# manycore-research/faceformer

Hardware: AMD Instinct MI355X
Metric: decoded edges/sec (greedy face-loop decode, pointer selections/s), 256-edge wireframes (higher is better)
Workload: dtype f32; 1 GPU; BASELINE config 2: configs/ours.yml model.num_lines=256: 1 synthetic 256-edge wireframe(s) per GPU, F=256 anchor sequences x 36 greedy steps, default-xavier synthetic weights; wireframes_per_gpu=1, edges=256, max_face_length=37, decode_steps=36, parallelism=wireframe-sharded x1, RCCL all-gather of predictions

## Files before the change

faceformer_amd/csrc/ff_common.h:

```cpp
#pragma once
#include <hip/hip_runtime.h>
#include <stdint.h>
#include <stdio.h>
#include <string.h>

#include "faceformer_hip.h"

#define FF_WAVE 64
#define FF_MAX_STREAMS 8

typedef float f32x4 __attribute__((ext_vector_type(4)));
typedef float f32x16 __attribute__((ext_vector_type(16)));

void ff_set_error(const char* fmt, ...);

#define FF_CHECK_ARG(cond, ...)           \
  do {                                    \
    if (!(cond)) {                        \
      ff_set_error(__VA_ARGS__);          \
      return FF_ERR_ARG;                  \
    }                                     \
  } while (0)

#define FF_CHECK_HIP(expr)                                                             \
// ... 57 lines not shown

size_t ff_attention_planes_stride();
bool ff_attention_x2h_ok(const ff_attn_desc& d);
int ff_attention_x2h_launch(const ff_attn_desc& d, const void* planes, long long plane_stride, hipStream_t st);

struct ff_pointer_sync {
  int* seen;
  int* arrive;
  int* host_slot;
  int host_which;
  float* next_stats;
  int logits_ready;
  const int* slot;
  int* fin;
  int fin_j, term_lo, term_hi;
};
int ff_pointer_argmax_sync(const float* p, int ldp, const float* memory, int S, int E, const unsigned char* mask,
                           const int* kv_len, const unsigned char* extra_mask, int ldextra, int B, int seqs_per_group,
                           int* next_tok, float* best, float* second, float* logprob, float* logits, int ldlogits,
                           float* next_rows, int ldnext, int* count_ge, int ge_bound, int* count_eq, int eq_value,
                           const ff_pointer_sync* sync, ff_stream_t stream);

int ff_beam_select_sync(float* logits, int ldlogits, int S, const unsigned char* mask, const int* kv_len, int groups, int width,
                        int groups_per_wireframe, const float* scores_in, float* scores_out, const int* fin_in, int* fin_out,
                        int* hist, int ldhist, int t, int* parent, int* next_tok, int term_lo, int term_hi, const float* memory,
                        int E, float* next_rows, int ldnext, int* count_ge, int ge_bound, float* next_stats, int* arrive,
                        int* host_slot, ff_stream_t stream);
int ff_beam_init(int* tok, float* score, int* fin, int* parent, int Bc, int Fc, int W, int f0, const int* num_input, int pad_tok,
                 int term_lo, int term_hi, hipStream_t st);
int ff_beam_finalize(const int* tok, const int* parent, const float* score, int Btot, int T, const int* steps_dev,
                     const int* num_input, int dedup, int F, int W, int w0, int nw, int Fc, int f0, int b0, int64_t* beams,
                     float* scores, int64_t* predict, int* seq_of_row, hipStream_t st);

int ff_forced_tokens(const int64_t* paths, int* tok, int rows, int T, int S, hipStream_t st);
int ff_forced_finalize(const int* tok, const float* lp_all, const int* greedy_all, const int* rank_all, const int* lengths, int rows,
                       int T, float* logprob, int64_t* greedy, int* rank, float* seq_logprob, hipStream_t st);
// ... 45 lines not shown
```

faceformer_amd/csrc/ff_device.h:

```cpp
#pragma once
#include "ff_common.h"

typedef float f32x2 __attribute__((ext_vector_type(2)));

#define FF_GLOBAL __attribute__((address_space(1)))
typedef unsigned long long ff_u64;

__device__ __forceinline__ f32x4 ff_ld16(const float* p) { return *reinterpret_cast<const f32x4*>(p); }
__device__ __forceinline__ f32x2 ff_ld8(const float* p) { return *reinterpret_cast<const f32x2*>(p); }
__device__ __forceinline__ float ff_ld4(const float* p) { return *p; }
__device__ __forceinline__ void ff_st16(float* p, f32x4 v) { *reinterpret_cast<f32x4*>(p) = v; }
__device__ __forceinline__ void ff_st8(float* p, f32x2 v) { *reinterpret_cast<f32x2*>(p) = v; }
__device__ __forceinline__ void ff_st4(float* p, float v) { *p = v; }
__device__ __forceinline__ int ff_ld4i(const int* p) { return *p; }
__device__ __forceinline__ void ff_st4i(int* p, int v) { *p = v; }
__device__ __forceinline__ void ff_store_tile(float* cp, int ldc, int row0, int col, int M, bool colok, const float (&v)[16]) {
  float* p = cp + (size_t)row0 * ldc + col;
  if (row0 - (row0 & 4) + 32 <= M) {
    if (colok) {
#pragma unroll
      for (int e = 0; e < 16; ++e) ff_st4(p + (size_t)((e & 3) + 8 * (e >> 2)) * ldc, v[e]);
    }
  } else {
#pragma unroll
// ... 597 lines not shown
  const float* memory; int S, E;
  const unsigned char* mask; const int* kv_len;
  const unsigned char* extra; int ldextra;
  int B, spg;
  int* next_tok; float* best; float* second; float* logits; int ldlogits;
  float* next_rows; int ldnext;
  int* count_ge; int ge_bound; int* count_eq; int eq_value;
  int* seen;
  int* arrive;
  int* host_slot;
  int host_which;
  float* next_stats;
  const int* slot;
  int* fin; int fin_j, term_lo, term_hi;
  float* logprob;
};
__device__ __forceinline__ int ff_pointer_seq(const PointerArgs& a, int b) { return a.slot ? a.slot[b] : b; }

__device__ __forceinline__ void ff_pointer_count_block(const PointerArgs& a, int b0, const int* toks, int nvalid) {
  int nge = 0, neq = 0;
  for (int i = 0; i < nvalid; ++i) {
    const int idx = toks[i];
    if (a.fin) {
      int* fp = a.fin + ff_pointer_seq(a, b0 + i);
      const int f = __hip_atomic_load(fp, __ATOMIC_RELAXED, __HIP_MEMORY_SCOPE_SYSTEM);
      if (f < a.fin_j) continue;
      if (idx >= a.term_lo && idx < a.term_hi) __hip_atomic_store(fp, a.fin_j, __ATOMIC_RELAXED, __HIP_MEMORY_SCOPE_SYSTEM);
    }
    if (a.count_ge && idx >= a.ge_bound) ++nge;
    if (a.count_eq && idx == a.eq_value) {
// ... 54 lines not shown
    const float ob1 = __shfl_xor(b1, off, FF_WAVE), ob2 = __shfl_xor(b2, off, FF_WAVE);
    const int oi1 = __shfl_xor(i1, off, FF_WAVE);
    if (LP) {
      const float om = __shfl_xor(lmax, off, FF_WAVE), os = __shfl_xor(lsum, off, FF_WAVE);
      lsum = ff_lse_merge(lmax, lsum, om, os, &lmax);
    }
    const bool other = (ob1 > b1) || (ob1 == b1 && oi1 < i1);
    const float nb2 = other ? fmaxf(ob2, b1) : fmaxf(b2, ob1);
    if (other) { b1 = ob1; i1 = oi1; }
    b2 = nb2;
  }
  if (i1 == 0x7fffffff) { i1 = 0; b1 = FILL; }
  *b1_out = b1; *b2_out = b2; *i1_out = i1; *lsum_out = lsum;
}

__device__ __forceinline__ void ff_pointer_append_row(const PointerArgs& a, int w, int b, int i1, int lane) {
  const float* src = a.memory + ((size_t)w * a.S + i1) * a.E;
  float* dst = a.next_rows + (size_t)b * a.ldnext;
  if (!a.next_stats) {
    for (int vi = lane; vi < (a.E >> 2); vi += 64)
      ff_st16(dst + vi * 4, ff_ldw16(src + vi * 4));
  } else {
    float* sdst = a.next_stats + (size_t)b * (a.E >> 5) * 2;
    for (int v0 = 0; v0 < (a.E >> 2); v0 += 64) {
      const int vi = v0 + lane;
      const bool in = vi < (a.E >> 2);
      f32x4 x = {0.f, 0.f, 0.f, 0.f};
      if (in) { x = ff_ldw16(src + vi * 4); ff_st16(dst + vi * 4, x); }
      float sm = (x.x + x.y) + (x.z + x.w);
      sm += __shfl_xor(sm, 1, FF_WAVE); sm += __shfl_xor(sm, 2, FF_WAVE); sm += __shfl_xor(sm, 4, FF_WAVE);
      const float mean = sm * (1.0f / 32.0f);
      const float d0 = x.x - mean, d1 = x.y - mean, d2 = x.z - mean, d3 = x.w - mean;
      float m2 = (d0 * d0 + d1 * d1) + (d2 * d2 + d3 * d3);
      m2 += __shfl_xor(m2, 1, FF_WAVE); m2 += __shfl_xor(m2, 2, FF_WAVE); m2 += __shfl_xor(m2, 4, FF_WAVE);
      if (in && (lane & 7) == 0) ff_st8(sdst + (vi >> 3) * 2, f32x2{mean, m2});
    }
  }
}

template <bool LP>
__device__ __forceinline__ int ff_pointer_reduce_row(const PointerArgs& a, int b, int lane) {
  float b1, b2, lsum;
  int i1;
  ff_pointer_mask_reduce<LP>(a, b, lane, &b1, &b2, &i1, &lsum);
  const int seq = ff_pointer_seq(a, b);
  if (lane == 0) {
    ff_st4i(a.next_tok + seq, i1);
    if (a.best) ff_st4(a.best + seq, b1);
    if (a.second) ff_st4(a.second + seq, b2);
    if (LP) ff_st4(a.logprob + seq, -logf(lsum));
  }
  if (a.next_rows) ff_pointer_append_row(a, b / a.spg, b, i1, lane);
  return i1;
}
```

faceformer_amd/csrc/ff_engine.hip:

```cpp
#include <chrono>
#include <cstdlib>
#include <mutex>
#include <vector>

#include "ff_common.h"
#include "ff_launch.h"

namespace {

struct Bump {
  char* base;
  size_t size, off;
  bool ok;
  Bump(void* p, size_t n) : base((char*)p), size(n), off(0), ok(true) {}
  template <typename T>
  T* take(size_t count) {
    size_t bytes = ff_align_up(count * sizeof(T), 256);
    if (off + bytes > size) { ok = false; off += bytes; return nullptr; }
    T* r = reinterpret_cast<T*>(base + off);
    off += bytes;
    return r;
  }
};

// ... 124 lines not shown
  g.row_table = d.table; g.ld_row_table = d.ldt; g.row_div = row_div; g.row_cols = d.tcols;
  g.ln_stats_out = d.st_out;
  if (split) return sk.ln(&g, d.planes, d.plane_rows, d.row0, d.st_in ? d.colsum : nullptr, st);
  return ff_gemm_f32_ln(&g, st);
}

struct Scratch {
  float *x, *y, *yq, *qkv, *o, *h, *p, *logits;
  float* lnstat;
};

struct DecodeBuffers {
  float *mem_pos, *kvc[FF_MAX_LAYERS];
  unsigned char* kvp[FF_MAX_LAYERS];
  float *x0_all, *qkv0_all;
  float* x0stat_all;
  float *projT, *pg_all, *pc_all;
  int* tok_all;
  float* lp_all;
  Scratch scr[FF_MAX_STREAMS];
  int* zeroed; size_t zeroed_count;
  int *cnt_ge, *cnt_eq;
  int *arrive;
  int *seen;
  int *cnt_tot;
  int *steps_dev;
  int *fin, *slot_all, *perm_all;
  float* bm_score;
  int *bm_fin, *bm_parent;
  float* fc_lp;
  int *fc_greedy, *fc_rank;
  float* sm_lp;
  int *sm_fin, *sm_row;
};

struct Chunk {
  int w0, nw, Fc, f0, b0, Bc, sid;
  int Fl, Bl;
  int *slot, *perm;
  float* x0;
  float* qkv0;
  float* x0stat;
  float *pg, *pc;
};

inline bool retiring(const ff_decode_params* p) { return p->variant == FF_PARALLEL && (p->flags & FF_RETIRE_FINISHED); }

inline int compact_width(const ff_decode_params* p, const int* num_input_host, int w) {
  if (p->variant != FF_PARALLEL || !(p->flags & FF_DEDUP_PAD_ANCHORS) || !num_input_host) return p->F;
  int n = num_input_host[w];
  n = n < 0 ? 0 : n;
  return n < p->F ? n + 1 : p->F;
}

void plan_chunks(const ff_decode_params* p, const int* num_input_host, int ns, std::vector<Chunk>* out, int* btot,
                 int* max_bc, int* nchunks = nullptr) {
  const int N = p->N;
// ... 64 lines not shown
  k.pinned = pc > 0 && pc < FF_PINNED_SLOTS ? pc : FF_PINNED_SLOTS;
  return k;
}

bool can_fuse_layernorm(const ff_model* m, const ff_decode_params* prm) {
  if (!(prm->flags & FF_FUSE_LAYERNORM)) return false;
  if (m->E % 64 != 0 || m->E < 128 || m->E > 512 || m->FF % 64 != 0 || m->FF < 128) return false;
  if (!m->proj_fold_w || !m->proj_fold_b) return false;
  for (int l = 0; l < m->num_dec_layers; ++l) {
    const ff_layer_weights& w = m->dec[l];
    if (!w.ln1_w || !w.ln1_b || !w.ln1_pos || !w.ln2_w || !w.ln2_b || !w.ln2_pos || !w.ln3_w || !w.ln3_b) return false;
  }
  return true;
}

size_t layout_decode(const ff_model* m, const ff_decode_params* p, const EngineKnobs& kn, size_t Btot, size_t Bch, size_t nch,
                     Bump& bp, DecodeBuffers* out, bool want_lp = false, bool beam = false, bool forced = false, bool sample = false) {
  const int E = m->E, FFd = m->FF, S = p->L + m->num_token, T = p->T;
  const int ns = plan_streams(p);
  const size_t Rmax = (size_t)(T - 1 > 0 ? T - 1 : 1) * Bch;
  DecodeBuffers b;
  memset(&b, 0, sizeof(b));
  b.mem_pos = bp.take<float>((size_t)p->N * S * E);
  for (int l = 0; l < m->num_dec_layers; ++l) b.kvc[l] = bp.take<float>((size_t)p->N * S * 2 * E);
  const bool planes = kn.x2h_attn && (m->split_kind == 1 || m->split_kind == 2) && p->x3_min_rows > 0 && S <= 288 && m->dec[0].in_proj_planes != nullptr;
  for (int l = 0; l < m->num_dec_layers; ++l)
    b.kvp[l] = planes ? bp.take<unsigned char>(ff_attention_planes_bytes(p->N, m->H)) : nullptr;
  b.x0_all = bp.take<float>((size_t)T * Btot * E);
  b.tok_all = bp.take<int>((size_t)T * Btot);
  b.qkv0_all = (p->flags & FF_REUSE_LAYER0_QKV) ? bp.take<float>((size_t)T * Btot * 3 * E) : nullptr;
  b.x0stat_all = (kn.l0_fold && (p->flags & FF_REUSE_LAYER0_QKV) && can_fuse_layernorm(m, p)) ? bp.take<float>(Btot * (size_t)(E / 32) * 2)
                                                                                 : nullptr;
  const bool pf = kn.pointer_fold && can_fuse_layernorm(m, p);
  b.projT = pf ? bp.take<float>((size_t)E * E) : nullptr;
  b.pg_all = pf ? bp.take<float>(nch * (size_t)S * E) : nullptr;
  b.pc_all = pf ? bp.take<float>(nch * (size_t)((S + 3) & ~3)) : nullptr;
  for (int s = 0; s < ns; ++s) {
    Scratch& c = b.scr[s];
    c.x = bp.take<float>(Rmax * E);
    c.y = bp.take<float>(Rmax * E);
    c.yq = bp.take<float>(Rmax * E);
    c.qkv = bp.take<float>(Rmax * 3 * E);
    c.o = bp.take<float>(Rmax * E);
    c.h = bp.take<float>(Rmax * FFd);
    c.p = bp.take<float>(Bch * E);
    c.logits = bp.take<float>(Bch * (size_t)S);
    c.lnstat = bp.take<float>(Rmax * (size_t)(E / 32 + 1) * 2);
  }
  const size_t ncnt = ff_align_up((size_t)T * nch * sizeof(int), 256) / sizeof(int);
  b.zeroed_count = 3 * ncnt + Btot;
  b.zeroed = bp.take<int>(b.zeroed_count);
// ... 47 lines not shown
  const bool prune_last = (prm->flags & FF_LAST_LAYER_LAST_ROW) != 0 && !full_rows;
  const bool fuse = step_fuses(m, prm, R);
  const int nseg = E / 32;
  const float* qpos = m->qpos_table;
  const float* qpos_new = qpos + (size_t)(t - 1) * E;
  auto proj = [&](const Proj& d) -> int { return project(m, prm, Bc, st, d); };
  const bool last_qkv_one = R <= kn.one_launch_rows;
  for (int l = 0; l < nd; ++l) {
    const ff_layer_weights& w = m->dec[l];
    const ff_mha_weights& sa = w.self_attn;
    const bool last = prune_last && (l == nd - 1);
    const float* xin = (l == 0) ? ck.x0 : buf.x;
    const float* QKV = buf.qkv;
    if (l == 0 && reuse0) {
      if (full_rows) {
      } else if (fuse && t > 1 && ck.x0stat) {
        FF_RETURN_IF(proj(Proj().in(xin + newoff * E, E).weight(w.ln1_w, E, w.ln1_b).norm(ck.x0stat)
                              .pos(w.ln1_pos + (size_t)(t - 1) * 2 * E, 2 * E, 2 * E).out(ck.qkv0 + newoff * 3 * E, 3 * E, Bc, 3 * E, E)));
      } else {
        FF_RETURN_IF(ff_layernorm(xin + newoff * E, E, w.norm1_w, w.norm1_b, m->ln_eps, buf.y, E, buf.yq, E,
                                  qpos_new, E, Bc, 1, Bc, E, st));
        FF_RETURN_IF(proj(Proj().in(buf.yq, E, buf.y, 2 * E).weight(sa.in_proj_w, E, sa.in_proj_b)
                              .out(ck.qkv0 + newoff * 3 * E, 3 * E, Bc, 3 * E, E)));
      }
      QKV = ck.qkv0;
    } else if (fuse && l > 0) {
      const bool kv_only = last && t > 1 && !last_qkv_one;
      const int c0 = kv_only ? E : 0;
      FF_RETURN_IF(proj(Proj().in(buf.x, E).weight(w.ln1_w + (size_t)c0 * E, E, w.ln1_b + c0).split(w.ln1_planes, 3 * E, c0, w.ln1_csum)
                            .norm(buf.lnstat).pos(w.ln1_pos + c0, 2 * E, 2 * E - c0).out(buf.qkv + c0, 3 * E, R, 3 * E - c0, E)));
// ... 209 lines not shown
    if (io.extra_mask || forced) prm.flags &= ~FF_DEDUP_PAD_ANCHORS;
    p = &prm;
    retire = retiring(p);
    dedup = p->variant == FF_PARALLEL && (p->flags & FF_DEDUP_PAD_ANCHORS) && io.num_input_host;
    each_eos = (p->flags & FF_STOP_EACH_EOS) != 0;
    kn = engine_knobs(p);
    return FF_OK;
  }
  int bind_chunks(void* workspace, size_t workspace_bytes) {
    const int ns_req = plan_streams(p);
    int max_bc = 0;
    if (W || R) plan_beam_chunks(p, io.num_input_host, ns_req, W ? W : R, &chunks, &Btot, &max_bc);
    else plan_chunks(p, io.num_input_host, ns_req, &chunks, &Btot, &max_bc);
    nch = (int)chunks.size();
    Bump bp(workspace, workspace_bytes);
    layout_decode(m, p, kn, (size_t)Btot, (size_t)max_bc, (size_t)nch, bp, &buf, io.logprob != nullptr, W > 0, forced != nullptr,
                  R > 0);
    if (!bp.ok) { ff_set_error("ff_decode: workspace too small (%zu needed, %zu given)", bp.off, workspace_bytes); return FF_ERR_WORKSPACE; }
    for (Chunk& c : chunks) {
      c.x0 = buf.x0_all + (size_t)T * c.b0 * E;
      c.qkv0 = buf.qkv0_all ? buf.qkv0_all + (size_t)T * c.b0 * 3 * E : nullptr;
      c.x0stat = buf.x0stat_all ? buf.x0stat_all + (size_t)c.b0 * (E / 32) * 2 : nullptr;
      const size_t ci = (size_t)(&c - chunks.data());
      const bool one = c.nw == 1 && buf.pg_all != nullptr;
      c.pg = one ? buf.pg_all + ci * (size_t)S * E : nullptr;
      c.pc = one ? buf.pc_all + ci * (size_t)((S + 3) & ~3) : nullptr;
      if (retire) { c.slot = buf.slot_all + c.b0; c.perm = buf.perm_all + c.b0; }
    }
    ns = ns_req < nch ? ns_req : nch;
    forked = ns > 1;
    lagged = (size_t)T * (size_t)nch <= (size_t)kn.pinned;
    fin_dev = buf.fin;
    slots_per_step.reserve((size_t)T);
    tot.reserve((size_t)T);
// ... 90 lines not shown
      }
    }
    FF_RETURN_IF(fork());
    bool any_pg = false;
    for (const Chunk& c : chunks) any_pg = any_pg || c.pg != nullptr;
    if (any_pg) {
      FF_RETURN_IF(ff_transpose(m->proj_fold_w, E, E, E, buf.projT, E, main_st));
      FF_RETURN_IF(fork());
      for (const Chunk& c : chunks) {
        if (!c.pg) continue;
        const float* mem_w = memory + (size_t)c.w0 * S * E;
        FF_RETURN_IF(gemm(mem_w, E, nullptr, 0, buf.projT, E, nullptr, nullptr, 0, c.pg, E, S, E, E, 0, sts[c.sid]));
        FF_RETURN_IF(gemm(mem_w, E, nullptr, 0, m->proj_fold_b, E, nullptr, nullptr, 0, c.pc, 1, S, 1, E, 0, sts[c.sid]));
      }
    }
    for (const Chunk& c : chunks) {
      if (forced) {
        FF_RETURN_IF(ff_gather_rows(memory + (size_t)c.w0 * S * E, S, E, buf.tok_all + c.b0, c.Bc, c.Fc, c.x0, E, sts[c.sid]));
        continue;
      }
      if (W) {
        FF_RETURN_IF(ff_beam_init(buf.tok_all + c.b0, buf.bm_score + c.b0, buf.bm_fin + c.b0, buf.bm_parent + c.b0, c.Bc, c.Fc / W, W,
                                  c.f0, io.num_input + c.w0, m->num_token - 1, p->term_lo, p->term_hi, sts[c.sid]));
        FF_RETURN_IF(ff_gather_rows(memory + (size_t)c.w0 * S * E, S, E, buf.tok_all + c.b0, c.Bc, c.Fc, c.x0, E, sts[c.sid]));
        continue;
      }
      if (R) {
        FF_RETURN_IF(ff_sample_init(buf.tok_all + c.b0, buf.sm_lp + c.b0, buf.sm_fin + c.b0, buf.sm_row + c.b0, c.Bc, c.Fc / R, R, c.f0,
                                    c.w0, F, io.num_input + c.w0, m->num_token - 1, p->term_lo, p->term_hi, sts[c.sid]));
        FF_RETURN_IF(ff_gather_rows(memory + (size_t)c.w0 * S * E, S, E, buf.tok_all + c.b0, c.Bc, c.Fc, c.x0, E, sts[c.sid]));
        continue;
      }
      hipLaunchKernelGGL(init_tokens_kernel, dim3(ff_cdiv(c.Bc, 256)), dim3(256), 0, sts[c.sid], buf.tok_all + c.b0,
                         c.Bc, c.Fc, c.f0, io.num_input ? io.num_input + c.w0 : nullptr, p->variant, m->num_token - 1,
                         p->tok_sos, c.slot, c.perm, c.slot ? c.Bl : 0);
      FF_CHECK_LAUNCH();
      if (c.Bl > 0)
        FF_RETURN_IF(ff_gather_rows(memory + (size_t)c.w0 * S * E, S, E, c.slot ? c.perm : buf.tok_all + c.b0, c.Bl, c.Fl, c.x0, E,
                                    sts[c.sid]));
    }
    return FF_OK;
  }
  int enqueue_step(int step) {
    const int t = step + 1;
    int nslots = 0;
    for (const Chunk& c : chunks) {
      if (c.Bl == 0) continue;
      nslots += c.Bl;
      hipStream_t st = sts[c.sid];
      const Scratch& sc = buf.scr[c.sid];
      const size_t trow = (size_t)step * ((size_t)N * F * (W ? W : (R ? R : 1))) + c.b0;
      const size_t slot = (size_t)step * nch + (size_t)(&c - chunks.data());
      const bool folded_head = c.pg != nullptr && step_fuses(m, p, (long)t * c.Bl);
      float* logits_dst = (io.trace_logits && !retire) ? io.trace_logits + trow * S : sc.logits;
      if (W) {
        FF_RETURN_IF(beam_step(c, sc, step, slot, folded_head, logits_dst, trow, st));
        continue;
      }
      if (R) {
        FF_RETURN_IF(sample_step(c, sc, step, slot, folded_head, logits_dst, st));
        continue;
      }
      ff_pointer_sync psync{each_eos ? buf.seen + c.b0 : nullptr, lagged ? buf.arrive + slot : nullptr,
                            lagged ? pool->hpin_dev + slot : nullptr, p->variant == FF_PARALLEL ? 0 : 1, c.x0stat,
                            folded_head ? 1 : 0, c.slot, retire ? fin_dev + c.b0 : nullptr, t, p->term_lo, p->term_hi};
      FF_RETURN_IF(decoder_pass(m, p, kn, buf, sc, c, c.Fl, c.Bl, io.mask, io.kv_len, t, false, nullptr, st,
                                folded_head ? logits_dst : nullptr));
      FF_RETURN_IF(ff_pointer_argmax_sync(
          folded_head ? nullptr : sc.p, E, io.memory + (size_t)c.w0 * S * E, S, E, io.mask + (size_t)c.w0 * S, io.kv_len + c.w0,
          io.extra_mask ? io.extra_mask + (size_t)c.b0 * S : nullptr, S, c.Bl, c.Fl,
          buf.tok_all + (size_t)t * Btot + c.b0, io.trace_best ? io.trace_best + trow : nullptr,
          io.trace_second ? io.trace_second + trow : nullptr,
          buf.lp_all ? buf.lp_all + (size_t)step * Btot + c.b0 : nullptr,
          logits_dst, S,
          c.x0 + (size_t)t * c.Bl * E, E, buf.cnt_ge + slot, m->num_token, buf.cnt_eq + slot, p->tok_eos,
          (each_eos || lagged || c.x0stat || folded_head || retire) ? &psync : nullptr, st));
      if (retire && io.trace_logits)
        FF_RETURN_IF(ff_permute_rows(sc.logits, c.Bl, nullptr, io.trace_logits + trow * S, c.Bc, c.slot, 1, c.Bl, S, st));
    }
    slots_per_step.push_back(nslots);
// ... 101 lines not shown
      for (int i = 0; i < nb; ++i) nhs[(size_t)i] = hs[(size_t)perm[(size_t)i]];
      if (nb > 0) {
        int* sp = pool->stage + soff;
        int* ss = sp + nb;
        soff += 2 * (size_t)nb;
        memcpy(sp, perm.data(), sizeof(int) * (size_t)nb);
        memcpy(ss, nhs.data(), sizeof(int) * (size_t)nb);
        FF_CHECK_HIP(hipMemcpyAsync(c.perm, sp, sizeof(int) * (size_t)nb, hipMemcpyHostToDevice, st));
        const Scratch& sc = buf.scr[c.sid];
        auto regather = [&](float* rows, float* scratch, int npos, int width) -> int {
          FF_RETURN_IF(ff_permute_rows(rows, c.Bl, c.perm, scratch, nb, nullptr, npos, nb, width, st));
          FF_CHECK_HIP(hipMemcpyAsync(rows, scratch, sizeof(float) * (size_t)npos * nb * width, hipMemcpyDeviceToDevice, st));
          return FF_OK;
        };
        FF_RETURN_IF(regather(c.x0, sc.x, enq + 1, E));
        if (c.qkv0) FF_RETURN_IF(regather(c.qkv0, sc.qkv, enq, 3 * E));
        if (c.x0stat) FF_RETURN_IF(regather(c.x0stat, sc.y, 1, E / 16));
        FF_CHECK_HIP(hipMemcpyAsync(c.slot, ss, sizeof(int) * (size_t)nb, hipMemcpyHostToDevice, st));
      }
      hs.swap(nhs);
      c.Fl = fl; c.Bl = nb;
    }
    return FF_OK;
  }
  int retire_at(int bound, bool drained) {
    if (fin_host) {
      const volatile int* v = fin_host;
      for (int i = 0; i < Btot; ++i) hfin[(size_t)i] = v[i];
    } else {
      FF_RETURN_IF(read_back(hfin.data(), buf.fin, (size_t)Btot, drained));
      bound = enq - 1;
// ... 157 lines not shown
    d.scale = 0.125f;
    FF_RETURN_IF(ff_attention(&d, st));
    FF_RETURN_IF(gemm(o, E, nullptr, 0, w.self_attn.out_w, E, w.self_attn.out_b, x, E, x, E, R, E, E, 0, st));
    FF_RETURN_IF(ff_layernorm(x, E, w.norm2_w, w.norm2_b, m->ln_eps, y, E, nullptr, 0, nullptr, 0, 1, 1, R, E, st));
    FF_RETURN_IF(gemm(y, E, nullptr, 0, w.lin1_w, E, w.lin1_b, nullptr, 0, hb, FFd, R, FFd, E, 1, st));
    FF_RETURN_IF(gemm(hb, FFd, nullptr, 0, w.lin2_w, FFd, w.lin2_b, x, E, x, E, R, E, FFd, 0, st));
  }
  FF_RETURN_IF(ff_layernorm(x, E, m->enc_norm_w, m->enc_norm_b, m->ln_eps, memory, E, nullptr, 0, nullptr, 0, 1, 1,
                            R, E, st));
  return FF_OK;
}

extern "C" size_t ff_decode_workspace_bytes(const ff_model* m, const ff_decode_params* p, const int* num_input_host) {
  if (!m || !p || p->N <= 0 || p->F <= 0 || p->T <= 0) return 0;
  int btot = 0, max_bc = 0, nch = 0;
  plan_chunks(p, num_input_host, 1, nullptr, &btot, &max_bc, &nch);
  Bump bp(nullptr, 0);
  return layout_decode(m, p, engine_knobs(p), (size_t)btot, (size_t)max_bc, (size_t)nch, bp, nullptr) + 256;
}

extern "C" size_t ff_decode_lp_workspace_bytes(const ff_model* m, const ff_decode_params* p, const int* num_input_host) {
  if (!m || !p || p->N <= 0 || p->F <= 0 || p->T <= 0) return 0;
  int btot = 0, max_bc = 0, nch = 0;
  plan_chunks(p, num_input_host, 1, nullptr, &btot, &max_bc, &nch);
  Bump bp(nullptr, 0);
  return layout_decode(m, p, engine_knobs(p), (size_t)btot, (size_t)max_bc, (size_t)nch, bp, nullptr, true) + 256;
}

extern "C" size_t ff_decode_beam_workspace_bytes(const ff_model* m, const ff_decode_params* p, const int* num_input_host, int width) {
  if (!m || !p || p->N <= 0 || p->F <= 0 || p->T <= 0 || width < 1 || width > 8) return 0;
  int btot = 0, max_bc = 0, nch = 0;
  plan_beam_chunks(p, num_input_host, 1, width, nullptr, &btot, &max_bc, &nch);
  Bump bp(nullptr, 0);
  return layout_decode(m, p, engine_knobs(p), (size_t)btot, (size_t)max_bc, (size_t)nch, bp, nullptr, false, true) + 256;
}

extern "C" int ff_decode(const ff_model* m, const ff_decode_params* p, const float* memory,
                         const unsigned char* mask, const int* kv_len, const int* num_input,
                         const int* num_input_host, const unsigned char* extra_mask, int64_t* predict,
                         int* steps_done, int* step_counts, float* pointer_out, float* trace_logits,
                         float* trace_best, float* trace_second, int* seq_of_row, void* workspace,
// ... 131 lines not shown
```

faceformer_amd/csrc/ff_gemm.hip:

```cpp
#include <stdlib.h>

#include "ff_common.h"
#include "ff_device.h"
#include "ff_launch.h"

namespace {


constexpr int LN_NQ = 2;
struct LnRaw { f32x2 seg[LN_NQ]; };
__device__ __forceinline__ void ff_ln_issue(const float* __restrict__ st, int nseg, int c, LnRaw& r) {
#pragma unroll
  for (int q = 0; q < LN_NQ; ++q) {
    const int sidx = c + 8 * q;
    r.seg[q] = ff_ld8(st + 2 * (sidx < nseg ? sidx : 0));
  }
}
__device__ __forceinline__ void ff_ln_finish(const LnRaw& r, int nseg, int c, float eps, float& mean, float& rstd) {
  float sm = 0.f, m2 = 0.f;
#pragma unroll
  for (int q = 0; q < LN_NQ; ++q)
    if (c + 8 * q < nseg) { sm += r.seg[q].x; m2 += r.seg[q].y; }
  sm = ff_sum8(sm);
  m2 = ff_sum8(m2);
// ... 1219 lines not shown
extern "C" int ff_set_gemm_tuning(int min_units, int two_per_cu_units, int fix_tenths, int small_max_rows) {
  FF_CHECK_ARG(min_units >= 1 && two_per_cu_units >= 1 && fix_tenths >= 0 && small_max_rows >= 0,
               "ff_set_gemm_tuning: bad arguments");
  g_sk_min_units.set(min_units);
  g_sk_two_per_cu.set(two_per_cu_units);
  g_sk_fix_tenths.set(fix_tenths);
  g_small_max_rows.set(small_max_rows);
  ff_tuning_changed();
  return FF_OK;
}

namespace {
inline long dma_min_rows() { return ff_knob(FF_K_DMA_MIN_ROWS); }
inline long dma_min_rows_n512() { return ff_knob(FF_K_DMA_MIN_ROWS_N512); }
inline long dma_min_rows_wide() { return ff_knob(FF_K_DMA_MIN_ROWS_WIDE); }
int gemm_dispatch(GemmArgs g, int batch, int tile, hipStream_t st) {
  const bool split128 = !g.A2 || (g.n_split % 128) == 0;
  if (tile == 0) tile = 7;
  if (tile == 5 && !split128) tile = 4;
  const int M = g.M, N = g.N, K = g.K;
  FFProfScope prof(FF_CAT_GEMM, 2.0 * M * N * K * batch, st);
  ff_prof_add_bytes(FF_CAT_GEMM, 4.0 * batch * ((double)M * K + (double)N * K + (double)M * N * (g.res ? 2 : 1)));
  const bool dma_ok = ff_gemm_dma_f32_ok(g, batch);
  if (tile == 11) {
    FF_CHECK_ARG(dma_ok, "ff_gemm_f32: tile 11 needs K %% 32 == 0, K >= 64, N %% 4 == 0, leading dimensions %% 4, 16-byte aligned operands, batch 1");
    return ff_gemm_dma_f32(g, st);
  }
  if (tile == 12) {
    FF_CHECK_ARG(dma_ok && (!g.A2 || (g.n_split % 64) == 0), "ff_gemm_f32: tile 12 needs what tile 11 needs");
    return ff_gemm_dma_f32(g, st, 64);
  }
  const long dmr = dma_min_rows(), dmr512 = dma_min_rows_n512(), dmrw = dma_min_rows_wide();
  const long dma_from = N <= 512 ? (dmr512 > dmr ? dmr512 : dmr) : (N >= 1536 && dmrw < dmr ? dmrw : dmr);
  if (tile == 7 && dma_ok && (long)M >= dma_from) return ff_gemm_dma_f32(g, st);
  switch (tile) {
    case 1: return launch_generic<64, 64, 32, 32>(g, batch, st);
    case 2: return launch_pipe<64, 64, 32, 32>(g, batch, st);
    case 3: return launch_persist(g, batch, st);
    case 4: return launch_pipe<128, 64, 64, 32>(g, batch, st);
    case 6: return launch_streamk(g, batch, st, 2);
    case 7:
      if (const int smr = g_small_max_rows.get(); (long)M * batch <= (N <= 512 ? smr : (smr * 3) / 4) && K >= 512 && small_ok(g))
        return launch_small(g, batch, st);
      if (batch == 1 && M >= 4096 && (K & 15) == 0 && gemm_mode(g) == 0 && (!g.A2 || (g.n_split & 63) == 0)) {
        const long t9 = (long)ff_cdiv(M, 128) * ff_cdiv(N, 64);
        const long rounds = (t9 + 511) / 512;
        if (10 * t9 >= 9 * rounds * 512) return launch_pipe<128, 64, 64, 32, 16>(g, batch, st);
      }
      return launch_streamk(g, batch, st, 0);
    case 8: FF_CHECK_ARG(small_ok(g), "ff_gemm_f32: tile 8 needs K in {128,256,512,1024}"); return launch_small(g, batch, st);
    case 9: return launch_pipe<128, 64, 64, 32, 16>(g, batch, st);
    case 10: return launch_pipe<128, 128, 64, 64, 16>(g, batch, st);
    default: return launch_pipe<128, 128, 64, 64>(g, batch, st);
  }
}
}

extern "C" int ff_gemm_f32_batched(const float* A, int lda, const float* A2, int n_split,
                                   const float* W, int ldw, const float* bias, const float* residual,
                                   int ldr, float* C, int ldc, int M, int N, int K, int act, int tile,
                                   int batch, long long stride_a, long long stride_w,
                                   long long stride_c, ff_stream_t stream) {
  if (M == 0 || N == 0 || batch == 0) return FF_OK;
  FF_CHECK_ARG(M > 0 && N > 0 && K > 0 && (K & 3) == 0, "ff_gemm_f32: bad M=%d N=%d K=%d (K %% 4)", M, N, K);
  FF_CHECK_ARG(A && W && C, "ff_gemm_f32: null operand");
  FF_CHECK_ARG((lda & 3) == 0 && (ldw & 3) == 0 && lda >= K && ldw >= K && ldc >= N,
               "ff_gemm_f32: bad leading dimensions lda=%d ldw=%d ldc=%d", lda, ldw, ldc);
  FF_CHECK_ARG(ff_aligned16(A) && ff_aligned16(W) && (!A2 || ff_aligned16(A2)),
               "ff_gemm_f32: A/A2/W must be 16-byte aligned");
  FF_CHECK_ARG(!residual || ldr >= N, "ff_gemm_f32: bad ldr");
// ... 48 lines not shown
```

faceformer_amd/csrc/ff_pointer.hip:

```cpp
#include <float.h>

#include "ff_common.h"
#include "ff_device.h"

namespace {


template <int NV, bool LP>
__device__ __forceinline__ int pointer_row(const PointerArgs& a, int b, int lane) {
  const int w = b / a.spg;
  const int nvec = a.E >> 2;
  f32x4 pv[NV];
#pragma unroll
  for (int c = 0; c < NV; ++c) {
    const int vi = lane + 64 * c;
    pv[c] = vi < nvec ? *reinterpret_cast<const f32x4*>(a.p + (size_t)b * a.ldp + vi * 4)
                      : f32x4{0.f, 0.f, 0.f, 0.f};
  }
  int kv = a.S;
  if (a.kv_len) { const int k = a.kv_len[w]; kv = k < kv ? k : kv; }
  const float* mem = a.memory + (size_t)w * a.S * a.E;
  const unsigned char* mrow = a.mask ? a.mask + (size_t)w * a.S : nullptr;
  const int seq = ff_pointer_seq(a, b);
  const unsigned char* erow = a.extra ? a.extra + (size_t)seq * a.ldextra : nullptr;
// ... 100 lines not shown
}

template <bool LP>
__global__ __launch_bounds__(256) void pointer_reduce_kernel(PointerArgs a) {
  __shared__ int s_tok[4];
  const int lane = threadIdx.x & 63;
  const int b = blockIdx.x * (blockDim.x >> 6) + (threadIdx.x >> 6);
  if (b < a.B) s_tok[threadIdx.x >> 6] = ff_pointer_reduce_row<LP>(a, b, lane);
  __syncthreads();
  if (threadIdx.x == 0) {
    const int b0 = blockIdx.x * (blockDim.x >> 6);
    ff_pointer_count_block(a, b0, s_tok, a.B - b0 < 4 ? a.B - b0 : 4);
  }
}

}

extern "C" int ff_pointer_argmax(const float* p, int ldp, const float* memory, int S, int E,
                                 const unsigned char* mask, const int* kv_len,
                                 const unsigned char* extra_mask, int ldextra, int B,
                                 int seqs_per_group, int* next_tok, float* best, float* second,
                                 float* logits, int ldlogits, float* next_rows, int ldnext,
                                 int* count_ge, int ge_bound, int* count_eq, int eq_value,
                                 ff_stream_t stream) {
  return ff_pointer_argmax_sync(p, ldp, memory, S, E, mask, kv_len, extra_mask, ldextra, B, seqs_per_group, next_tok, best,
                                second, nullptr, logits, ldlogits, next_rows, ldnext, count_ge, ge_bound, count_eq, eq_value,
                                nullptr, stream);
}

extern "C" int ff_pointer_argmax_lp(const float* p, int ldp, const float* memory, int S, int E,
// ... 9 lines not shown
}

int ff_pointer_argmax_sync(const float* p, int ldp, const float* memory, int S, int E, const unsigned char* mask,
                           const int* kv_len, const unsigned char* extra_mask, int ldextra, int B, int seqs_per_group,
                           int* next_tok, float* best, float* second, float* logprob, float* logits, int ldlogits,
                           float* next_rows, int ldnext, int* count_ge, int ge_bound, int* count_eq, int eq_value,
                           const ff_pointer_sync* sync, ff_stream_t stream) {
  if (B == 0) return FF_OK;
  FF_CHECK_ARG(B > 0 && S > 0 && E > 0 && (E & 3) == 0 && E <= 2048 && seqs_per_group > 0,
               "ff_pointer_argmax: bad sizes B=%d S=%d E=%d", B, S, E);
  const bool logits_ready = sync && sync->logits_ready;
  FF_CHECK_ARG((p || logits_ready) && memory && next_tok, "ff_pointer_argmax: null pointer");
  FF_CHECK_ARG(!logits_ready || (logits && (B % seqs_per_group) == 0), "ff_pointer_argmax: logits_ready without a logits buffer");
  FF_CHECK_ARG(!(sync && sync->next_stats) || (logits && (B % seqs_per_group) == 0 && (E & 31) == 0),
               "ff_pointer_argmax: next_stats needs the GEMM path (a logits buffer) and E %% 32 == 0");
  FF_CHECK_ARG((logits_ready && !p) || ((ldp & 3) == 0 && ff_aligned16(p)), "ff_pointer_argmax: p misaligned");
  FF_CHECK_ARG(ff_aligned16(memory), "ff_pointer_argmax: memory misaligned");
  FF_CHECK_ARG(!next_rows || ((ldnext & 3) == 0 && ff_aligned16(next_rows)), "ff_pointer_argmax: next_rows misaligned");
  FF_CHECK_ARG(!logits || ldlogits >= S, "ff_pointer_argmax: ldlogits < S");
  FF_CHECK_ARG(!extra_mask || ldextra >= S, "ff_pointer_argmax: ldextra < S");
  PointerArgs a{p, ldp, memory, S, E, mask, kv_len, extra_mask, ldextra, B, seqs_per_group,
                next_tok, best, second, logits, ldlogits, next_rows, ldnext,
                count_ge, ge_bound, count_eq, eq_value,
                sync ? sync->seen : nullptr, sync ? sync->arrive : nullptr, sync ? sync->host_slot : nullptr,
                sync ? sync->host_which : 0, sync ? sync->next_stats : nullptr,
                sync ? sync->slot : nullptr, sync ? sync->fin : nullptr, sync ? sync->fin_j : 0,
                sync ? sync->term_lo : 0, sync ? sync->term_hi : 0, logprob};
  FF_CHECK_ARG(!a.arrive || (a.host_slot && (a.host_which ? count_eq : count_ge)), "ff_pointer_argmax: counter hand-over without a counter");
  hipStream_t st = (hipStream_t)stream;
  dim3 grid(ff_cdiv(B, 4)), block(256);
  if (logits != nullptr && (B % seqs_per_group) == 0) {
    if (!logits_ready)
      FF_RETURN_IF(ff_gemm_f32_batched(p, ldp, nullptr, 0, memory, E, nullptr, nullptr, 0, logits, ldlogits,
                                       seqs_per_group, S, E, 0, 0, B / seqs_per_group,
                                       (long long)seqs_per_group * ldp, (long long)S * E,
                                       (long long)seqs_per_group * ldlogits, stream));
    FFProfScope prof(FF_CAT_POINTER, (double)B * S * 8.0, st);
    if (logprob) hipLaunchKernelGGL(pointer_reduce_kernel<true>, grid, block, 0, st, a);
    else hipLaunchKernelGGL(pointer_reduce_kernel<false>, grid, block, 0, st, a);
    FF_CHECK_LAUNCH();
    return FF_OK;
  }
// ... 15 lines not shown
```

faceformer_amd/hip/engine.py:

```python
import ctypes as C

import torch

from . import lib as _L
from .ops import SPLIT_KINDS, _dev, _p, _stream, split_weight

import operator

_VERSION_OF = operator.attrgetter("_version")

RETIRE_MIN_SHRINK = 0.125

DEFAULT_FLAGS = (_L.FF_REUSE_LAYER0_QKV | _L.FF_LAST_LAYER_LAST_ROW | _L.FF_DEDUP_PAD_ANCHORS
                 | _L.FF_FUSE_LAYERNORM)


def _kv_len_from_mask(mask_u8):
    S = mask_u8.size(1)
    idx = torch.arange(1, S + 1, device=mask_u8.device, dtype=torch.int32)
    return ((mask_u8 == 0).to(torch.int32) * idx).amax(dim=1).to(torch.int32).contiguous()


FP16_LIM = 6.0e4
ATTN_Q_SCALE = 0.125 * 1.4426950408889634


def fp16_operand_bounds(tensors, n_dec, E, weights=0.0):
    root = float(E) ** 0.5

# ... 495 lines not shown
```

faceformer_amd/hip/lib.py:

```python
import ctypes as C
import os

HERE = os.path.dirname(os.path.abspath(__file__))
LIB_PATH = os.environ.get("FF_HIP_LIB") or os.path.join(HERE, "libfaceformer_hip.so")

FF_MAX_LAYERS = 16
FF_HEAD_DIM = 64
FF_PARALLEL, FF_SEQ2SEQ = 0, 1
FF_REUSE_LAYER0_QKV, FF_LAST_LAYER_LAST_ROW, FF_RETURN_POINTER, FF_NO_STOP, FF_DEDUP_PAD_ANCHORS = 1, 2, 4, 8, 16
FF_FUSE_LAYERNORM = 32
FF_STOP_EACH_EOS = 512
FF_NO_L0_FOLD = 1024
FF_NO_POINTER_FOLD = 2048
FF_RETIRE_FINISHED = 4096
FF_ABI_VERSION = 105

fptr = C.c_void_p


class HipExtensionError(RuntimeError):
    pass


class AttnDesc(C.Structure):
    _fields_ = [
        ("q", fptr), ("k", fptr), ("v", fptr), ("o", fptr),
        ("ldq", C.c_int), ("ldk", C.c_int), ("ldv", C.c_int), ("ldo", C.c_int),
        ("num_groups", C.c_int), ("num_heads", C.c_int),
        ("nq", C.c_int),
# ... 249 lines not shown
```

include/faceformer_hip.h:

```cpp
#ifndef FACEFORMER_HIP_H
#define FACEFORMER_HIP_H

#include <stddef.h>
#include <stdint.h>

#ifdef __cplusplus
extern "C" {
#endif

typedef void* ff_stream_t;

enum ff_status {
  FF_OK = 0,
  FF_ERR_ARG = -1,
  FF_ERR_LAUNCH = -2,
  FF_ERR_WORKSPACE = -3,
  FF_ERR_NO_DEVICE = -4
};

#define FF_HEAD_DIM 64
#define FF_MAX_LAYERS 16

#define FF_ABI_VERSION 105
int ff_version(void);
// ... 194 lines not shown
int ff_encode(const ff_model* m, const float* input, const unsigned char* mask, const int* kv_len,
              int N, int L, float* memory, void* workspace, size_t workspace_bytes,
              ff_stream_t stream);

enum ff_variant { FF_PARALLEL = 0, FF_SEQ2SEQ = 1 };
enum ff_decode_flags {
  FF_REUSE_LAYER0_QKV = 1,
  FF_LAST_LAYER_LAST_ROW = 2,
  FF_RETURN_POINTER = 4,
  FF_NO_STOP = 8,
  FF_FUSE_LAYERNORM = 32,
  FF_DEDUP_PAD_ANCHORS = 16,
  FF_NO_L0_FOLD = 1024,
  FF_NO_POINTER_FOLD = 2048,
  FF_RETIRE_FINISHED = 4096,
  FF_STOP_EACH_EOS = 512
};

typedef int (*ff_stop_fn)(void* user, const int* step_counts, int num_steps);

typedef struct ff_decode_params {
  int variant;
  int N;
  int L;
  int F;
  int T;
  int chunk_wireframes;
  int chunk_seqs;
  int num_streams;
  int sync_every;
// ... 95 lines not shown
```

Baseline: 158,000 edges/s.

## Precompute layer-0 QKV table over memory rows and gather it in pointer kernel

Precomputes the layer-0 layernormed QKV projection for every memory row (S rows per wireframe) once before the greedy decode loop. The pointer argmax kernel then copies the selected row's QKV into the next step's qkv0 buffer and adds the positional term. This replaces the per-step layer-0 projection GEMM for new tokens. The cost is an upfront table GEMM, a stats kernel and extra workspace. The table is only enabled when S rows per wireframe is no more than the rows projected over all steps, and it is on by default through DEFAULT_FLAGS.

New measurement: 158,700 edges/s, median of 6. Within noise of the previous version (+0.5%).

```diff
diff --git a/faceformer_amd/csrc/ff_common.h b/faceformer_amd/csrc/ff_common.h
--- a/faceformer_amd/csrc/ff_common.h
+++ b/faceformer_amd/csrc/ff_common.h
@@ -95,12 +95,19 @@
   const int* slot;
   int* fin;
   int fin_j, term_lo, term_hi;
+  const float* tab0;
+  const float* pos0;
+  float* next_qkv;
 };
 int ff_pointer_argmax_sync(const float* p, int ldp, const float* memory, int S, int E, const unsigned char* mask,
                            const int* kv_len, const unsigned char* extra_mask, int ldextra, int B, int seqs_per_group,
                            int* next_tok, float* best, float* second, float* logprob, float* logits, int ldlogits,
                            float* next_rows, int ldnext, int* count_ge, int ge_bound, int* count_eq, int eq_value,
                            const ff_pointer_sync* sync, ff_stream_t stream);
+
+int ff_row_segment_stats(const float* x, int ldx, int rows, int E, float* stats, hipStream_t st);
+
+int ff_gemm_f32_rows_of_same_form(int M, int N, int K);
 
 int ff_beam_select_sync(float* logits, int ldlogits, int S, const unsigned char* mask, const int* kv_len, int groups, int width,
                         int groups_per_wireframe, const float* scores_in, float* scores_out, const int* fin_in, int* fin_out,
diff --git a/faceformer_amd/csrc/ff_device.h b/faceformer_amd/csrc/ff_device.h
--- a/faceformer_amd/csrc/ff_device.h
+++ b/faceformer_amd/csrc/ff_device.h
@@ -635,6 +635,7 @@
   const int* slot;
   int* fin; int fin_j, term_lo, term_hi;
   float* logprob;
+  const float* tab0; const float* pos0; float* next_qkv;
 };
 __device__ __forceinline__ int ff_pointer_seq(const PointerArgs& a, int b) { return a.slot ? a.slot[b] : b; }
 
@@ -719,6 +720,16 @@
   *b1_out = b1; *b2_out = b2; *i1_out = i1; *lsum_out = lsum;
 }
 
+__device__ __forceinline__ f32x2 ff_segment_stats(f32x4 x) {
+  float sm = (x.x + x.y) + (x.z + x.w);
+  sm += __shfl_xor(sm, 1, FF_WAVE); sm += __shfl_xor(sm, 2, FF_WAVE); sm += __shfl_xor(sm, 4, FF_WAVE);
+  const float mean = sm * (1.0f / 32.0f);
+  const float d0 = x.x - mean, d1 = x.y - mean, d2 = x.z - mean, d3 = x.w - mean;
+  float m2 = (d0 * d0 + d1 * d1) + (d2 * d2 + d3 * d3);
+  m2 += __shfl_xor(m2, 1, FF_WAVE); m2 += __shfl_xor(m2, 2, FF_WAVE); m2 += __shfl_xor(m2, 4, FF_WAVE);
+  return f32x2{mean, m2};
+}
+
 __device__ __forceinline__ void ff_pointer_append_row(const PointerArgs& a, int w, int b, int i1, int lane) {
   const float* src = a.memory + ((size_t)w * a.S + i1) * a.E;
   float* dst = a.next_rows + (size_t)b * a.ldnext;
@@ -732,13 +743,29 @@
       const bool in = vi < (a.E >> 2);
       f32x4 x = {0.f, 0.f, 0.f, 0.f};
       if (in) { x = ff_ldw16(src + vi * 4); ff_st16(dst + vi * 4, x); }
-      float sm = (x.x + x.y) + (x.z + x.w);
-      sm += __shfl_xor(sm, 1, FF_WAVE); sm += __shfl_xor(sm, 2, FF_WAVE); sm += __shfl_xor(sm, 4, FF_WAVE);
-      const float mean = sm * (1.0f / 32.0f);
-      const float d0 = x.x - mean, d1 = x.y - mean, d2 = x.z - mean, d3 = x.w - mean;
-      float m2 = (d0 * d0 + d1 * d1) + (d2 * d2 + d3 * d3);
-      m2 += __shfl_xor(m2, 1, FF_WAVE); m2 += __shfl_xor(m2, 2, FF_WAVE); m2 += __shfl_xor(m2, 4, FF_WAVE);
-      if (in && (lane & 7) == 0) ff_st8(sdst + (vi >> 3) * 2, f32x2{mean, m2});
+      const f32x2 st = ff_segment_stats(x);
+      if (in && (lane & 7) == 0) ff_st8(sdst + (vi >> 3) * 2, st);
+    }
+  }
+}
+
+__device__ __forceinline__ void ff_pointer_append_qkv0(const PointerArgs& a, int w, int b, int i1, int lane) {
+  constexpr int NB = 6;
+  const int nvec = 3 * (a.E >> 2), npos = a.E >> 1;
+  const float* src = a.tab0 + ((size_t)w * a.S + i1) * 3 * a.E;
+  float* dst = a.next_qkv + (size_t)b * 3 * a.E;
+  for (int v0 = lane; v0 < nvec; v0 += 64 * NB) {
+    f32x4 v[NB], pv[NB];
+#pragma unroll
+    for (int i = 0; i < NB; ++i) {
+      const int vi = v0 + 64 * i;
+      if (vi < nvec) v[i] = ff_ld16(src + vi * 4);
+      if (vi < npos) pv[i] = ff_ldw16(a.pos0 + vi * 4);
+    }
+#pragma unroll
+    for (int i = 0; i < NB; ++i) {
+      const int vi = v0 + 64 * i;
+      if (vi < nvec) ff_st16(dst + vi * 4, vi < npos ? v[i] + pv[i] : v[i]);
     }
   }
 }
@@ -756,5 +783,6 @@
     if (LP) ff_st4(a.logprob + seq, -logf(lsum));
   }
   if (a.next_rows) ff_pointer_append_row(a, b / a.spg, b, i1, lane);
+  if (a.tab0) ff_pointer_append_qkv0(a, b / a.spg, b, i1, lane);
   return i1;
 }
diff --git a/faceformer_amd/csrc/ff_engine.hip b/faceformer_amd/csrc/ff_engine.hip
--- a/faceformer_amd/csrc/ff_engine.hip
+++ b/faceformer_amd/csrc/ff_engine.hip
@@ -162,6 +162,7 @@
   float *mem_pos, *kvc[FF_MAX_LAYERS];
   unsigned char* kvp[FF_MAX_LAYERS];
   float *x0_all, *qkv0_all;
+  float* tab0_all;
   float* x0stat_all;
   float *projT, *pg_all, *pc_all;
   int* tok_all;
@@ -189,6 +190,7 @@
   float* x0;
   float* qkv0;
   float* x0stat;
+  float* tab0;
   float *pg, *pc;
 };
 
@@ -283,8 +285,18 @@
   return true;
 }
 
+inline bool l0_table_here(const ff_decode_params* p, const Chunk& c, int S) {
+  return (p->flags & FF_L0_TABLE) && (long)c.nw * S <= (long)c.Bc * (p->T - 1);
+}
+size_t l0_table_rows(const ff_decode_params* p, const std::vector<Chunk>& chunks, int S) {
+  size_t rows = 0;
+  for (const Chunk& c : chunks) rows += l0_table_here(p, c, S) ? (size_t)c.nw * S : 0;
+  return rows;
+}
+
 size_t layout_decode(const ff_model* m, const ff_decode_params* p, const EngineKnobs& kn, size_t Btot, size_t Bch, size_t nch,
-                     Bump& bp, DecodeBuffers* out, bool want_lp = false, bool beam = false, bool forced = false, bool sample = false) {
+                     Bump& bp, DecodeBuffers* out, bool want_lp = false, bool beam = false, bool forced = false, bool sample = false,
+                     size_t tab_rows = 0) {
   const int E = m->E, FFd = m->FF, S = p->L + m->num_token, T = p->T;
   const int ns = plan_streams(p);
   const size_t Rmax = (size_t)(T - 1 > 0 ? T - 1 : 1) * Bch;
@@ -298,12 +310,13 @@
   b.x0_all = bp.take<float>((size_t)T * Btot * E);
   b.tok_all = bp.take<int>((size_t)T * Btot);
   b.qkv0_all = (p->flags & FF_REUSE_LAYER0_QKV) ? bp.take<float>((size_t)T * Btot * 3 * E) : nullptr;
-  b.x0stat_all = (kn.l0_fold && (p->flags & FF_REUSE_LAYER0_QKV) && can_fuse_layernorm(m, p)) ? bp.take<float>(Btot * (size_t)(E / 32) * 2)
-                                                                                 : nullptr;
+  const bool l0_fold = kn.l0_fold && (p->flags & FF_REUSE_LAYER0_QKV) && can_fuse_layernorm(m, p);
+  b.x0stat_all = l0_fold ? bp.take<float>(Btot * (size_t)(E / 32) * 2) : nullptr;
   const bool pf = kn.pointer_fold && can_fuse_layernorm(m, p);
   b.projT = pf ? bp.take<float>((size_t)E * E) : nullptr;
   b.pg_all = pf ? bp.take<float>(nch * (size_t)S * E) : nullptr;
   b.pc_all = pf ? bp.take<float>(nch * (size_t)((S + 3) & ~3)) : nullptr;
+  b.tab0_all = (tab_rows && l0_fold) ? bp.take<float>(tab_rows * 3 * E) : nullptr;
   for (int s = 0; s < ns; ++s) {
     Scratch& c = b.scr[s];
     c.x = bp.take<float>(Rmax * E);
@@ -381,6 +394,7 @@
     const float* QKV = buf.qkv;
     if (l == 0 && reuse0) {
       if (full_rows) {
+      } else if (fuse && t > 1 && ck.x0stat && ck.tab0) {
       } else if (fuse && t > 1 && ck.x0stat) {
         FF_RETURN_IF(proj(Proj().in(xin + newoff * E, E).weight(w.ln1_w, E, w.ln1_b).norm(ck.x0stat)
                               .pos(w.ln1_pos + (size_t)(t - 1) * 2 * E, 2 * E, 2 * E).out(ck.qkv0 + newoff * 3 * E, 3 * E, Bc, 3 * E, E)));
@@ -620,10 +634,13 @@
     else plan_chunks(p, io.num_input_host, ns_req, &chunks, &Btot, &max_bc);
     nch = (int)chunks.size();
     Bump bp(workspace, workspace_bytes);
+    const bool greedy = !W && !R && !forced;
     layout_decode(m, p, kn, (size_t)Btot, (size_t)max_bc, (size_t)nch, bp, &buf, io.logprob != nullptr, W > 0, forced != nullptr,
-                  R > 0);
+                  R > 0, greedy ? l0_table_rows(p, chunks, S) : 0);
     if (!bp.ok) { ff_set_error("ff_decode: workspace too small (%zu needed, %zu given)", bp.off, workspace_bytes); return FF_ERR_WORKSPACE; }
+    size_t tab_off = 0;
     for (Chunk& c : chunks) {
+      if (buf.tab0_all && l0_table_here(p, c, S)) { c.tab0 = buf.tab0_all + tab_off * 3 * E; tab_off += (size_t)c.nw * S; }
       c.x0 = buf.x0_all + (size_t)T * c.b0 * E;
       c.qkv0 = buf.qkv0_all ? buf.qkv0_all + (size_t)T * c.b0 * 3 * E : nullptr;
       c.x0stat = buf.x0stat_all ? buf.x0stat_all + (size_t)c.b0 * (E / 32) * 2 : nullptr;
@@ -744,6 +761,7 @@
         FF_RETURN_IF(gemm(mem_w, E, nullptr, 0, m->proj_fold_b, E, nullptr, nullptr, 0, c.pc, 1, S, 1, E, 0, sts[c.sid]));
       }
     }
+    FF_RETURN_IF(build_l0_tables());
     for (const Chunk& c : chunks) {
       if (forced) {
         FF_RETURN_IF(ff_gather_rows(memory + (size_t)c.w0 * S * E, S, E, buf.tok_all + c.b0, c.Bc, c.Fc, c.x0, E, sts[c.sid]));
@@ -768,6 +786,27 @@
       if (c.Bl > 0)
         FF_RETURN_IF(ff_gather_rows(memory + (size_t)c.w0 * S * E, S, E, c.slot ? c.perm : buf.tok_all + c.b0, c.Bl, c.Fl, c.x0, E,
                                     sts[c.sid]));
+    }
+    return FF_OK;
+  }
+  int build_l0_tables() {
+    const int nseg = E / 32;
+    const ff_layer_weights& w = m->dec[0];
+    for (Chunk& c : chunks) {
+      if (!c.tab0) continue;
+      const int rows = c.nw * S;
+      if (c.Bl == 0 || c.Bl > rows || (long)rows > (long)c.Bl * (T - 1)) { c.tab0 = nullptr; continue; }
+      hipStream_t st = sts[c.sid];
+      const float* mem_w = io.memory + (size_t)c.w0 * S * E;
+      float* stat = buf.scr[c.sid].lnstat;
+      FF_RETURN_IF(ff_row_segment_stats(mem_w, E, rows, E, stat, st));
+      const int like = ff_gemm_f32_rows_of_same_form(c.Bl, 3 * E, E);
+      const int M = like < rows ? like : rows;
+      for (int r0 = 0; r0 < rows; r0 += M) {
+        const size_t r = (size_t)(r0 + M <= rows ? r0 : rows - M);
+        FF_RETURN_IF(project(m, p, M, st, Proj().in(mem_w + r * E, E).weight(w.ln1_w, E, w.ln1_b).norm(stat + r * nseg * 2)
+                                              .out(c.tab0 + r * 3 * E, 3 * E, M, 3 * E, E)));
+      }
     }
     return FF_OK;
   }
@@ -793,7 +832,9 @@
       }
       ff_pointer_sync psync{each_eos ? buf.seen + c.b0 : nullptr, lagged ? buf.arrive + slot : nullptr,
                             lagged ? pool->hpin_dev + slot : nullptr, p->variant == FF_PARALLEL ? 0 : 1, c.x0stat,
-                            folded_head ? 1 : 0, c.slot, retire ? fin_dev + c.b0 : nullptr, t, p->term_lo, p->term_hi};
+                            folded_head ? 1 : 0, c.slot, retire ? fin_dev + c.b0 : nullptr, t, p->term_lo, p->term_hi,
+                            c.tab0, c.tab0 ? m->dec[0].ln1_pos + (size_t)t * 2 * E : nullptr,
+                            c.tab0 ? c.qkv0 + (size_t)t * c.Bl * 3 * E : nullptr};
       FF_RETURN_IF(decoder_pass(m, p, kn, buf, sc, c, c.Fl, c.Bl, io.mask, io.kv_len, t, false, nullptr, st,
                                 folded_head ? logits_dst : nullptr));
       FF_RETURN_IF(ff_pointer_argmax_sync(
@@ -925,7 +966,7 @@
           return FF_OK;
         };
         FF_RETURN_IF(regather(c.x0, sc.x, enq + 1, E));
-        if (c.qkv0) FF_RETURN_IF(regather(c.qkv0, sc.qkv, enq, 3 * E));
+        if (c.qkv0) FF_RETURN_IF(regather(c.qkv0, sc.qkv, c.tab0 ? enq + 1 : enq, 3 * E));
         if (c.x0stat) FF_RETURN_IF(regather(c.x0stat, sc.y, 1, E / 16));
         FF_CHECK_HIP(hipMemcpyAsync(c.slot, ss, sizeof(int) * (size_t)nb, hipMemcpyHostToDevice, st));
       }
@@ -1113,17 +1154,21 @@
 extern "C" size_t ff_decode_workspace_bytes(const ff_model* m, const ff_decode_params* p, const int* num_input_host) {
   if (!m || !p || p->N <= 0 || p->F <= 0 || p->T <= 0) return 0;
   int btot = 0, max_bc = 0, nch = 0;
-  plan_chunks(p, num_input_host, 1, nullptr, &btot, &max_bc, &nch);
+  std::vector<Chunk> chunks;
+  plan_chunks(p, num_input_host, 1, &chunks, &btot, &max_bc, &nch);
   Bump bp(nullptr, 0);
-  return layout_decode(m, p, engine_knobs(p), (size_t)btot, (size_t)max_bc, (size_t)nch, bp, nullptr) + 256;
+  return layout_decode(m, p, engine_knobs(p), (size_t)btot, (size_t)max_bc, (size_t)nch, bp, nullptr, false, false, false, false,
+                       l0_table_rows(p, chunks, p->L + m->num_token)) + 256;
 }
 
 extern "C" size_t ff_decode_lp_workspace_bytes(const ff_model* m, const ff_decode_params* p, const int* num_input_host) {
   if (!m || !p || p->N <= 0 || p->F <= 0 || p->T <= 0) return 0;
   int btot = 0, max_bc = 0, nch = 0;
-  plan_chunks(p, num_input_host, 1, nullptr, &btot, &max_bc, &nch);
+  std::vector<Chunk> chunks;
+  plan_chunks(p, num_input_host, 1, &chunks, &btot, &max_bc, &nch);
   Bump bp(nullptr, 0);
-  return layout_decode(m, p, engine_knobs(p), (size_t)btot, (size_t)max_bc, (size_t)nch, bp, nullptr, true) + 256;
+  return layout_decode(m, p, engine_knobs(p), (size_t)btot, (size_t)max_bc, (size_t)nch, bp, nullptr, true, false, false, false,
+                       l0_table_rows(p, chunks, p->L + m->num_token)) + 256;
 }
 
 extern "C" size_t ff_decode_beam_workspace_bytes(const ff_model* m, const ff_decode_params* p, const int* num_input_host, int width) {
diff --git a/faceformer_amd/csrc/ff_gemm.hip b/faceformer_amd/csrc/ff_gemm.hip
--- a/faceformer_amd/csrc/ff_gemm.hip
+++ b/faceformer_amd/csrc/ff_gemm.hip
@@ -1257,6 +1257,10 @@
 inline long dma_min_rows() { return ff_knob(FF_K_DMA_MIN_ROWS); }
 inline long dma_min_rows_n512() { return ff_knob(FF_K_DMA_MIN_ROWS_N512); }
 inline long dma_min_rows_wide() { return ff_knob(FF_K_DMA_MIN_ROWS_WIDE); }
+inline long dma_from_rows(int N) {
+  const long dmr = dma_min_rows(), dmr512 = dma_min_rows_n512(), dmrw = dma_min_rows_wide();
+  return N <= 512 ? (dmr512 > dmr ? dmr512 : dmr) : (N >= 1536 && dmrw < dmr ? dmrw : dmr);
+}
 int gemm_dispatch(GemmArgs g, int batch, int tile, hipStream_t st) {
   const bool split128 = !g.A2 || (g.n_split % 128) == 0;
   if (tile == 0) tile = 7;
@@ -1273,8 +1277,7 @@
     FF_CHECK_ARG(dma_ok && (!g.A2 || (g.n_split % 64) == 0), "ff_gemm_f32: tile 12 needs what tile 11 needs");
     return ff_gemm_dma_f32(g, st, 64);
   }
-  const long dmr = dma_min_rows(), dmr512 = dma_min_rows_n512(), dmrw = dma_min_rows_wide();
-  const long dma_from = N <= 512 ? (dmr512 > dmr ? dmr512 : dmr) : (N >= 1536 && dmrw < dmr ? dmrw : dmr);
+  const long dma_from = dma_from_rows(N);
   if (tile == 7 && dma_ok && (long)M >= dma_from) return ff_gemm_dma_f32(g, st);
   switch (tile) {
     case 1: return launch_generic<64, 64, 32, 32>(g, batch, st);
@@ -1297,6 +1300,18 @@
     default: return launch_pipe<128, 128, 64, 64>(g, batch, st);
   }
 }
+}
+
+int ff_gemm_f32_rows_of_same_form(int M, int N, int K) {
+  if (M <= 0 || N <= 0 || !(K == 512 || K == 1024)) return M;
+  const int smr = g_small_max_rows.get();
+  long lim = N <= 512 ? smr : (smr * 3) / 4;
+  if (lim >= dma_from_rows(N)) lim = dma_from_rows(N) - 1;
+  if (M > lim) return M;
+  const long tn = ff_cdiv(N, 32);
+  if ((long)ff_cdiv(M, 32) * tn > g_small_wide_blocks) return (int)lim;
+  const long wide_rows = 32 * (g_small_wide_blocks / tn);
+  return (int)(wide_rows < lim ? wide_rows : lim);
 }
 
 extern "C" int ff_gemm_f32_batched(const float* A, int lda, const float* A2, int n_split,
diff --git a/faceformer_amd/csrc/ff_pointer.hip b/faceformer_amd/csrc/ff_pointer.hip
--- a/faceformer_amd/csrc/ff_pointer.hip
+++ b/faceformer_amd/csrc/ff_pointer.hip
@@ -138,6 +138,33 @@
   }
 }
 
+__global__ __launch_bounds__(256) void row_segment_stats_kernel(const float* __restrict__ x, int ldx, int rows, int E,
+                                                                float* __restrict__ stats) {
+  const int lane = threadIdx.x & 63;
+  const int r = blockIdx.x * (blockDim.x >> 6) + (threadIdx.x >> 6);
+  if (r >= rows) return;
+  const float* src = x + (size_t)r * ldx;
+  float* sdst = stats + (size_t)r * (E >> 5) * 2;
+  for (int v0 = 0; v0 < (E >> 2); v0 += 64) {
+    const int vi = v0 + lane;
+    const bool in = vi < (E >> 2);
+    f32x4 v = {0.f, 0.f, 0.f, 0.f};
+    if (in) v = ff_ldw16(src + vi * 4);
+    const f32x2 st = ff_segment_stats(v);
+    if (in && (lane & 7) == 0) ff_st8(sdst + (vi >> 3) * 2, st);
+  }
+}
+
+}
+
+int ff_row_segment_stats(const float* x, int ldx, int rows, int E, float* stats, hipStream_t st) {
+  if (rows == 0) return FF_OK;
+  FF_CHECK_ARG(x && stats && rows > 0 && E > 0 && (E & 31) == 0 && (ldx & 3) == 0 && ldx >= E && ff_aligned16(x),
+               "ff_row_segment_stats: bad arguments rows=%d E=%d ldx=%d", rows, E, ldx);
+  FFProfScope prof(FF_CAT_ROWOP, (double)rows * E * 4.0, st);
+  hipLaunchKernelGGL(row_segment_stats_kernel, dim3(ff_cdiv(rows, 4)), dim3(256), 0, st, x, ldx, rows, E, stats);
+  FF_CHECK_LAUNCH();
+  return FF_OK;
 }
 
 extern "C" int ff_pointer_argmax(const float* p, int ldp, const float* memory, int S, int E,
@@ -177,6 +204,10 @@
   FF_CHECK_ARG(!logits_ready || (logits && (B % seqs_per_group) == 0), "ff_pointer_argmax: logits_ready without a logits buffer");
   FF_CHECK_ARG(!(sync && sync->next_stats) || (logits && (B % seqs_per_group) == 0 && (E & 31) == 0),
                "ff_pointer_argmax: next_stats needs the GEMM path (a logits buffer) and E %% 32 == 0");
+  const bool tab = sync && sync->tab0;
+  FF_CHECK_ARG(!tab || (logits && (B % seqs_per_group) == 0 && sync->next_qkv && sync->pos0 && ff_aligned16(sync->tab0) &&
+                        ff_aligned16(sync->pos0) && ff_aligned16(sync->next_qkv)),
+               "ff_pointer_argmax: the layer-0 table needs the GEMM path (a logits buffer), pos0 and next_qkv, 16-byte aligned");
   FF_CHECK_ARG((logits_ready && !p) || ((ldp & 3) == 0 && ff_aligned16(p)), "ff_pointer_argmax: p misaligned");
   FF_CHECK_ARG(ff_aligned16(memory), "ff_pointer_argmax: memory misaligned");
   FF_CHECK_ARG(!next_rows || ((ldnext & 3) == 0 && ff_aligned16(next_rows)), "ff_pointer_argmax: next_rows misaligned");
@@ -188,7 +219,8 @@
                 sync ? sync->seen : nullptr, sync ? sync->arrive : nullptr, sync ? sync->host_slot : nullptr,
                 sync ? sync->host_which : 0, sync ? sync->next_stats : nullptr,
                 sync ? sync->slot : nullptr, sync ? sync->fin : nullptr, sync ? sync->fin_j : 0,
-                sync ? sync->term_lo : 0, sync ? sync->term_hi : 0, logprob};
+                sync ? sync->term_lo : 0, sync ? sync->term_hi : 0, logprob,
+                tab ? sync->tab0 : nullptr, tab ? sync->pos0 : nullptr, tab ? sync->next_qkv : nullptr};
   FF_CHECK_ARG(!a.arrive || (a.host_slot && (a.host_which ? count_eq : count_ge)), "ff_pointer_argmax: counter hand-over without a counter");
   hipStream_t st = (hipStream_t)stream;
   dim3 grid(ff_cdiv(B, 4)), block(256);
diff --git a/faceformer_amd/hip/engine.py b/faceformer_amd/hip/engine.py
--- a/faceformer_amd/hip/engine.py
+++ b/faceformer_amd/hip/engine.py
@@ -12,7 +12,7 @@
 RETIRE_MIN_SHRINK = 0.125
 
 DEFAULT_FLAGS = (_L.FF_REUSE_LAYER0_QKV | _L.FF_LAST_LAYER_LAST_ROW | _L.FF_DEDUP_PAD_ANCHORS
-                 | _L.FF_FUSE_LAYERNORM)
+                 | _L.FF_FUSE_LAYERNORM | _L.FF_L0_TABLE)
 
 
 def _kv_len_from_mask(mask_u8):
diff --git a/faceformer_amd/hip/lib.py b/faceformer_amd/hip/lib.py
--- a/faceformer_amd/hip/lib.py
+++ b/faceformer_amd/hip/lib.py
@@ -13,6 +13,7 @@
 FF_NO_L0_FOLD = 1024
 FF_NO_POINTER_FOLD = 2048
 FF_RETIRE_FINISHED = 4096
+FF_L0_TABLE = 8192
 FF_ABI_VERSION = 105
 
 fptr = C.c_void_p
diff --git a/include/faceformer_hip.h b/include/faceformer_hip.h
--- a/include/faceformer_hip.h
+++ b/include/faceformer_hip.h
@@ -232,6 +232,7 @@
   FF_NO_L0_FOLD = 1024,
   FF_NO_POINTER_FOLD = 2048,
   FF_RETIRE_FINISHED = 4096,
+  FF_L0_TABLE = 8192,
   FF_STOP_EACH_EOS = 512
 };
 
```
